# AI4Science-WestlakeU/cindm

Measured on AMD Instinct MI355X. Metric: design samples/sec (1000-step DDPM, composed U-Nets); rel-err vs CPU ref, higher is better.
Workload: dtype f32; 1 GPU; nbody-2 TemporalUnet1D dim=64 horizon=24 attention, single model, batch 256/GPU, 1000 DDPM steps per design (BASELINE configs[1]); unet_evals_per_design=1000, reverse_steps_per_design=1000, parallelism=dp1 (design-sharded, one all-gather of final designs)

## Files before the change

cindm_amd/csrc/cindm_hip.hip:

```cpp
#include "kernels.h"
#include "kernels_dconv.h"
#include "kernels2d.h"
#include "kernels2d_v2.h"
#include "../../include/cindm_hip.h"

#include <hip/hip_ext.h>
#include <cmath>
#include <cstdio>
#include <cstdlib>
#include <cstring>
#include <map>
#include <mutex>
#include <string>
#include <unordered_map>
#include <vector>

using namespace cindm;

static thread_local std::string g_err;
static int fail(const std::string& m) { g_err = m; return -1; }
#define HIPCHK(x) do { hipError_t e_ = (x); if (e_ != hipSuccess) return fail(std::string(#x) + ": " + hipGetErrorString(e_)); } while (0)
#define REQUIRE(c, msg) do { if (!(c)) return fail(msg); } while (0)

extern "C" int cindm_abi_version(void) { return CINDM_ABI_VERSION; }
// ... 120 lines not shown
    }
    const int mid = h->dims[nres];
    rtb("mid_block1", mid, mid);
    if (d.attention) attn("mid_attn", mid);
    rtb("mid_block2", mid, mid);
    cblock("final_conv.0", dim, dim);
    conv("final_conv.1", dim, d.transition_dim, 1);
    return 0;
}

static const OptDef kUnet1dOpts[] = {
    {"mfma_f32", 0, nullptr, OPT_PACK},
    {"local_gn", 1, "CINDM_LOCAL_GN", OPT_PACK},
    {"attn_site", 1, "CINDM_ATTN_SITE", OPT_PACK},
    {"level0", 1, "CINDM_LEVEL0", OPT_PACK},
    {"level1", 1, "CINDM_LEVEL1", OPT_PACK},
    {"ups_last", 1, "CINDM_UPS_LAST", OPT_PACK},
    {"ups_tail", 1, "CINDM_UPS_TAIL", OPT_PACK},
    {"attn_head", 1, "CINDM_ATTN_HEAD", OPT_PACK},
    {"dconv", 1, "CINDM_DCONV", OPT_PACK},
    {"ws_alias", 1, "CINDM_WS_ALIAS", OPT_PACK},
    {"pingpong", 1, "CINDM_PINGPONG", OPT_PACK},
    {"dresample", 2, "CINDM_DRESAMPLE", OPT_PACK},
    {"dconv2", 1, "CINDM_DCONV2", OPT_PACK},
    {"l2_prefetch", 1, "CINDM_L2_PREFETCH", OPT_PACK},
    {"fuse_gather", 1, nullptr, OPT_PACK},
    {"fuse_update", 1, "CINDM_FUSE_UPDATE", OPT_PACK},
    {"taps", 0, "CINDM_TAPS", OPT_PACK},
    {"recover", 1, nullptr, OPT_RUNTIME},
    {"no_exchange", 0, "CINDM_NO_EXCHANGE", OPT_RUNTIME},
    {"tune", 0, "CINDM_TUNE", OPT_RUNTIME},
    {"stress", 0, "CINDM_STRESS", OPT_PACK},
    {"auto_range", 1, "CINDM_AUTO_RANGE", OPT_PACK},
    {"range_fallback", 0, nullptr, OPT_READONLY},
    {"dbg", 0, "CINDM_DBG", OPT_PACK},
};

static void unet1d_plan(cindm_unet1d* h);
extern "C" int cindm_unet1d_set_option(cindm_unet1d* h, const char* key, int32_t value) {
    const int rc = core_set_option(h, key, value);
    if (rc == 1) {
        h->generation = ++g_generation;
        if (std::string(key) == "tune" && h->finalized) unet1d_plan(h);
    }
    return rc < 0 ? -1 : 0;
}
// ... 578 lines not shown
            else DC(3, 4, 0, false);
        }
#undef DC
    }
    E.prof_end();
    hipError_t e = hipGetLastError();
    if (e != hipSuccess && E.err == hipSuccess) E.err = e;
}

static bool dconv_applicable(cindm_unet1d* h, const std::string& p, const Ten& x0, const Ten* x1, int cout) {
    if (!h->O("dconv") || !h->use_h3 || !h->O("local_gn")) return false;
    const int L = x0.L, gw = cout / 8;
    if ((L != 3 && L != 6) || cout % 32 || (gw != 16 && gw != 32 && gw != 64)) return false;
    if (gw == 64 && ((cout / 32) % 2 || h->NX())) return false;
    if (x0.C % 128 || (x1 && (x1->C % 128 || x1->L != L))) return false;
    if (x0.ld != x0.C || (x1 && x1->ld != x1->C)) return false;
    auto w0 = h->packed.find(p + ".blocks.0.block.0"), w1 = h->packed.find(p + ".blocks.1.block.0");
    if (w0 == h->packed.end() || w1 == h->packed.end() || !w0->second.h3 || !w1->second.h3) return false;
    const bool identity = !h->packed.count(p + ".residual_conv");
    if (!identity && !h->packed.count(p + ".residual_conv#h3")) return false;
    const int k0 = x0.C / 128, k1 = x1 ? x1->C / 128 : 0;
    if (w0->second.CinP != (k0 + k1) * 128 || w1->second.CinP != cout || cout % 128) return false;
    return dconv_instantiated(L, k0, k1, !identity) && dconv_instantiated(L, cout / 128, 0, false);
}

static bool dconv2_instantiated(int L, int k0, int k1, bool res, int kb) {
    if (L == 6) return kb == 2 && ((k0 == 1 && k1 == 0 && res) || (k0 == 2 && k1 == 0 && !res) || (k0 == 2 && k1 == 2 && res));
    if (L == 3) return (kb == 4 && ((k0 == 2 && k1 == 0 && res) || (k0 == 4 && k1 == 0 && !res) || (k0 == 4 && k1 == 4 && res))) ||
                       (kb == 2 && k0 == 4 && k1 == 0 && res);
    return false;
}

static Ten emit_rtb_dconv2(Emitter& E, const std::string& p, const Ten& x0, const Ten* x1, int cout) {
    cindm_unet1d* h = E.h;
    const int Bp = (int)E.rows, L = x0.L, S = 48 / L, gw = cout / 8, NT = cout / 32;
    const int tiles = (Bp + S - 1) / S;
    const Packed& w0 = h->packed.at(p + ".blocks.0.block.0");
    const Packed& w1 = h->packed.at(p + ".blocks.1.block.0");
    const bool identity = !h->packed.count(p + ".residual_conv");
    const int k0 = x0.C / 128, k1 = x1 ? x1->C / 128 : 0, kb = cout / 128;
    Ten y0; y0.L = L; y0.C = cout; y0.ld = cout; E.planes(y0);
    Ten out = E.ten(L, cout); E.planes(out);
    unsigned long long* fl = E.xchg((size_t)tiles * NT);
    unsigned long long* xa = gw == 64 ? E.xchg((size_t)tiles * NT * 32) : nullptr;
    unsigned long long* xb = gw == 64 ? E.xchg((size_t)tiles * NT * 32) : nullptr;
    E.need_epoch();
// ... 185 lines not shown
        Emitter::plain(a.src[0], x0);
        if (identity) { a.res = x0.p; a.ldres = x0.ld; } else { a.res = r.p; a.ldres = r.ld; }
    }
    a.e_y = y1.p; a.e_ld = y1.ld; a.e_stats = st1; a.e_P = Pn; a.e_gw = gw; a.e_cnt = cnt;
    a.e_gamma = E.V(p + ".blocks.1.block.2.weight"); a.e_beta = E.V(p + ".blocks.1.block.2.bias");
    a.out = out.p; a.ldo = out.ld;
    if (want_ln) { *ln_out = E.alloc((size_t)Bp * L * (ceil_to(cout, TN) / TN) * 2); a.ln_out = *ln_out; }
    E.launch((identity || fused_res) ? 0 : 1, a);
    E.drop(y0); E.drop(y1); E.drop(k0); E.drop(k1);
    if (fused_res) E.drop(r);
    E.tap(p, out);
    return out;
}

static Ten emit_attn(Emitter& E, const std::string& p, const Ten& x, const float* lnp) {
    cindm_unet1d* h = E.h;
    const int Bp = (int)E.rows, L = x.L, C = x.C;
    const Packed& wq = h->packed.at(p + ".fn.fn.to_qkv");
    const Packed& wo = h->packed.at(p + ".fn.fn.to_out");
    GemmArgs a;
    auto site = h->packed.find(p + ".fn.fn.to_qkv#site");
    if (site != h->packed.end() && site->second.h3 && h->O("attn_head") && !h->NX() && (C == 512 || (C == 256 && (L <= 4 || h->O("attn_head") > 1))) && L <= 16 && x.ld == C) {
        Ten out = E.ten(L, C);
        const int slot = ceil_to(L, 4), S = 16 / slot, groups = (Bp + S - 1) / S;
        unsigned long long* xg = E.xchg((size_t)groups * 2048);
        E.need_epoch();
        ++E.launches;
        Pf pfs;
        E.pf_issue = false;
        E.pf_all(pfs, {&site->second, &h->packed.at(p + ".fn.fn.to_out#site")}, {});
        E.pf_issue = true;
        if (!E.dry) {
            AttnHeadArgs s;
            std::memset(&s, 0, sizeof(s));
            s.pf = pfs;
            s.x = x.p; s.ldx = x.ld; s.out = out.p; s.ldo = out.ld; s.g = E.V(p + ".fn.norm.g");
            s.Wqkv = E.W(site->second); s.Wo = E.W(h->packed.at(p + ".fn.fn.to_out#site")); s.bo = E.B(h->packed.at(p + ".fn.fn.to_out"));
            s.L = L; s.S = S; s.slot = slot; s.Bp = Bp;
            s.xchg = xg; s.epoch = h->ep(); s.err_flag = h->epoch_dev + 1;
            s.stress = h->O("stress");
            s.ph = E.ph_next("attn1d_head<" + std::to_string(C) + "> " + p);
            const dim3 grid(4, (unsigned)groups);
            E.prof_begin(5, 2.0 * Bp * L * 1024.0 * C + (double)Bp * 4 * (2.0 * 32 * 32 * L * 2));
            for (int rep = 0; rep < (E.prof ? Emitter::prof_reps : 1); ++rep) {
                if (C == 256) KLAUNCH(E, attn1d_head_kernel<256>, grid, dim3(256), 0, s);
                else KLAUNCH(E, attn1d_head_kernel<512>, grid, dim3(256), 0, s);
            }
            E.prof_end();
            hipError_t e = hipGetLastError();
            if (e != hipSuccess && E.err == hipSuccess) E.err = e;
        }
        E.tap(p, out);
        return out;
    }
    if (site != h->packed.end() && L <= 32) {
        Ten out = E.ten(L, C);
        ++E.launches;
        Pf pfs;
        E.pf_all(pfs, {&site->second, &h->packed.at(p + ".fn.fn.to_out#site")}, {});
        if (!E.dry) {
            AttnSiteArgs s;
            s.pf = pfs;
            s.x = x.p; s.ldx = x.ld; s.out = out.p; s.ldo = out.ld; s.g = E.V(p + ".fn.norm.g");
            s.Wqkv = E.W(site->second); s.Wo = E.W(h->packed.at(p + ".fn.fn.to_out#site")); s.bo = E.B(h->packed.at(p + ".fn.fn.to_out"));
            s.L = L; s.Bp = Bp;
            s.dbg = 0;
            s.ph = site->second.h3 ? E.ph_next("attn1d_site<" + std::to_string(C) + "> " + p) : PhaseBuf{nullptr, 0};
            const int pack = 1;
            const int NTsel = (L > 16) ? 2 : 1;
            s.slot = (L > 16) ? 32 : ceil_to(L, 4);
            s.S = (L > 16 || !pack) ? 1 : 16 / s.slot;
            const dim3 grid((unsigned)((Bp + s.S - 1) / s.S));
            E.prof_begin(5, 2.0 * Bp * L * 1024.0 * C + (double)Bp * 4 * (2.0 * 32 * 32 * L * 2));
            for (int rep = 0; rep < (E.prof ? Emitter::prof_reps : 1); ++rep) {
#define SITE_LAUNCH(C_, NT_, PF_) KLAUNCH(E, (attn1d_site_kernel<C_, NT_, PF_>), grid, dim3(256), 0, s)
#define SITE_LAUNCH_H3(C_, NT_, PF_) KLAUNCH(E, (attn1d_site_h3_kernel<C_, NT_, PF_>), grid, dim3(256), 0, s)
                if (site->second.h3) {
                    if (NTsel == 2) {
                        if (C == 64) SITE_LAUNCH_H3(64, 2, 2); else if (C == 128) SITE_LAUNCH_H3(128, 2, 3);
                        else if (C == 256) SITE_LAUNCH_H3(256, 2, 3); else SITE_LAUNCH_H3(512, 2, 3);
                    } else {
                        if (C == 64) SITE_LAUNCH_H3(64, 1, 2); else if (C == 128) SITE_LAUNCH_H3(128, 1, 3);
                        else if (C == 256) SITE_LAUNCH_H3(256, 1, 3); else SITE_LAUNCH_H3(512, 1, 3);
                    }
                } else if (NTsel == 2) {
                    if (C == 64) SITE_LAUNCH(64, 2, 4); else if (C == 128) SITE_LAUNCH(128, 2, 4);
                    else if (C == 256) SITE_LAUNCH(256, 2, 4); else SITE_LAUNCH(512, 2, 4);
                } else {
                    if (C == 64) SITE_LAUNCH(64, 1, 4); else if (C == 128) SITE_LAUNCH(128, 1, 4);
// ... 67 lines not shown
    E.tap(p, out);
    return out;
}

static Ten emit_resample(Emitter& E, const std::string& p, const Ten& x, bool up) {
    cindm_unet1d* h = E.h;
    const Packed& w = h->packed.at(p + ".conv");
    const int Lout = up ? x.L * 2 : x.L / 2;
    Ten out = E.ten(Lout, x.C);
    if (h->O("dresample") && h->O("dconv") && w.h3 && x.C == 256 && x.ld == x.C && x.L == (up ? 3 : 6) && w.CinP == x.C && w.T == (up ? 4 : 3)) {
        const int Bp = (int)E.rows, NT = x.C / 32, tiles = (Bp + 15) / 16;
        E.planes(out);
        ++E.launches;
        const bool half = h->O("dresample") >= 2 && NT % 8 == 0 && NT * tiles < 256 && !h->NX();
        int XS = 2;
        while (XS >= 1 && XS < 8 && tiles % (8 / XS) != 0) XS *= 2;
        if (!(XS == 2 || XS == 4) || (half ? 2 * NT : NT) % XS != 0 || (h->O("tune") & 1)) XS = 0;
        Pf pf;
        E.pf_tiled(pf, w, NT);
        if (!E.dry) {
            DresArgs d;
            std::memset(&d, 0, sizeof(d));
            d.pf = pf;
            d.x = x.p; d.ld = x.ld; d.W = reinterpret_cast<const uint4*>(E.W(w)); d.bias = E.B(w); d.nch = w.CinP / 128;
            d.Bp = Bp; d.N = x.C; d.NT = NT; d.out_f32 = out.p; d.ldo = out.ld; d.out_planes = out.pl; d.out_pstride = out.pst;
            d.ph = E.ph_next(std::string("dresample<") + (up ? "up" : "down") + "> " + p);
            d.xs = XS;
            const dim3 grid((unsigned)(half ? 2 * NT : NT), (unsigned)tiles);
            E.prof_begin(up ? 3 : 2, 2.0 * Bp * Lout * x.C * (double)x.C * (up ? 2.0 : 3.0));
            if (E.prof) { E.prof->back().gx = grid.x; E.prof->back().gy = grid.y; E.prof->back().nstage = d.nch; }
            if (half) {
                if (up) KLAUNCH(E, (dresample_kernel<true, 2, 2>), grid, dim3(256), 0, d);
                else KLAUNCH(E, (dresample_kernel<false, 2, 2>), grid, dim3(256), 0, d);
            } else {
                if (up) KLAUNCH(E, (dresample_kernel<true, 2, 1>), grid, dim3(256), 0, d);
                else KLAUNCH(E, (dresample_kernel<false, 2, 1>), grid, dim3(256), 0, d);
            }
            E.prof_end();
            hipError_t e = hipGetLastError();
            if (e != hipSuccess && E.err == hipSuccess) E.err = e;
        }
        E.tap(p, out);
        return out;
    }
    GemmArgs a;
    E.base(a, w, (int)E.rows, x.L, Lout);
    a.pad = 1;
// ... 60 lines not shown
                l.t_ptr = E.t_ptr; l.t_imm = E.t_imm; l.L = L;
                l.ph = E.ph_next("level0_down downs.0");
                E.prof_begin(5, 0.0);
                for (int rep = 0; rep < (E.prof ? Emitter::prof_reps : 1); ++rep) {
                    if (L > 16 && E.rows > 320) KLAUNCH(E, (level0_down_kernel<2, 2>), dim3((unsigned)E.rows), dim3(256), 0, l);
                    else if (L > 16) KLAUNCH(E, level0_down_kernel<2>, dim3((unsigned)E.rows), dim3(256), 0, l);
                    else KLAUNCH(E, level0_down_kernel<1>, dim3((unsigned)E.rows), dim3(256), 0, l);
                }
                E.prof_end();
            }
            if (taps) { E.tap("downs.0.0", h1); E.tap("downs.0.1", h2); }
            E.tap("downs.0.2", sk); E.tap("downs.0.3", dn);
            skips.push_back(sk);
            move_to(dn);
            continue;
        }
        const int lvl1 = h->O("level1");
        if (ind == 1 && lvl1 && h->level1_ok && att && cur.L <= 16 && (cur.L & 1) == 0 && cur.C == 64 && cur.ld == 64 &&
            h->packed.count("downs.1.2.fn.fn.to_qkv#site") && h->packed.at("downs.1.2.fn.fn.to_qkv#site").h3) {
            const int L = cur.L;
            Ten h1, h2;
            if (taps) { h1 = E.ten(L, 128); h2 = E.ten(L, 128); }
            Ten sk = E.ten(L, 128), dn = E.ten(L / 2, 128);
            ++E.launches;
            Pf pfl;
            E.pf_all(pfl, {&h->packed.at("downs.1.0.blocks.0.block.0#lvl"), &h->packed.at("downs.1.0.blocks.1.block.0#lvl"),
                           &h->packed.at("downs.1.1.blocks.0.block.0#lvl"), &h->packed.at("downs.1.1.blocks.1.block.0#lvl"),
                           &h->packed.at("downs.1.0.residual_conv#lvl"), &h->packed.at("downs.1.3.conv#lvl")},
                     {&h->packed.at("downs.1.2.fn.fn.to_qkv#site"), &h->packed.at("downs.1.2.fn.fn.to_out#site")});
            if (!E.dry) {
                Level1Args l;
                std::memset(&l, 0, sizeof(l));
                l.pf = pfl;
                l.x = cur.p; l.h1 = taps ? h1.p : nullptr; l.h2 = taps ? h2.p : nullptr; l.skip = sk.p; l.down = dn.p;
                const char* cv[4] = {"downs.1.0.blocks.0", "downs.1.0.blocks.1", "downs.1.1.blocks.0", "downs.1.1.blocks.1"};
                for (int i = 0; i < 4; ++i) {
                    const std::string cp = cv[i];
                    l.Wc[i] = E.W(h->packed.at(cp + ".block.0#lvl")); l.bc[i] = E.B(h->packed.at(cp + ".block.0"));
                    l.gam[i] = E.V(cp + ".block.2.weight"); l.bet[i] = E.V(cp + ".block.2.bias");
                }
                l.Wr = E.W(h->packed.at("downs.1.0.residual_conv#lvl")); l.br = E.B(h->packed.at("downs.1.0.residual_conv"));
                l.tb0 = h->ttable + h->tb_off.at("downs.1.0"); l.tb1 = h->ttable + h->tb_off.at("downs.1.1"); l.tb_ld = h->tb_ld;
                l.ln_g = E.V("downs.1.2.fn.norm.g"); l.Wqkv = E.W(h->packed.at("downs.1.2.fn.fn.to_qkv#site"));
                l.Wo = E.W(h->packed.at("downs.1.2.fn.fn.to_out#site")); l.bo = E.B(h->packed.at("downs.1.2.fn.fn.to_out"));
                l.Wd = E.W(h->packed.at("downs.1.3.conv#lvl")); l.bd = E.B(h->packed.at("downs.1.3.conv"));
                l.t_ptr = E.t_ptr; l.t_imm = E.t_imm; l.L = L; l.Bp = (int)E.rows;
                l.dbg = 0;
                l.ph = E.ph_next("level1_down downs.1");
                const int S = lvl1 == 1 ? 1 : 2;
                const dim3 grid((unsigned)((E.rows + S - 1) / S));
                E.prof_begin(5, 0.0);
                for (int rep = 0; rep < (E.prof ? Emitter::prof_reps : 1); ++rep) {
                    if (S == 1 && E.rows > 320) KLAUNCH(E, (level1_down_kernel<1, 2>), grid, dim3(256), 0, l);
                    else if (S == 1) KLAUNCH(E, level1_down_kernel<1>, grid, dim3(256), 0, l);
                    else KLAUNCH(E, level1_down_kernel<2>, grid, dim3(256), 0, l);
                }
                E.prof_end();
            }
            if (taps) { E.tap("downs.1.0", h1); E.tap("downs.1.1", h2); }
            E.tap("downs.1.2", sk); E.tap("downs.1.3", dn);
            skips.push_back(sk);
            move_to(dn);
            continue;
        }
        move_to(emit_rtb(E, p + ".0", cur, nullptr, co, false, nullptr));
        move_to(emit_rtb(E, p + ".1", cur, nullptr, co, need_ln(p + ".2", cur.L), &lnp));
        if (att) move_to(emit_attn(E, p + ".2", cur, lnp));
        skips.push_back(cur);
        cur_is_skip = true;
        if (h->packed.count(p + ".3.conv")) move_to(emit_resample(E, p + ".3", cur, false));
// ... 1248 lines not shown
```

cindm_amd/csrc/kernels.h:

```cpp
#pragma once
#include <hip/hip_runtime.h>
#include <stdint.h>
#include <type_traits>

namespace cindm {

typedef float f32x4 __attribute__((ext_vector_type(4)));

__device__ __forceinline__ void permlane16_pair(float v, float& a, float& b) {
    a = v; b = v;
    asm volatile("s_nop 1\n\tv_permlane16_swap_b32_e32 %0, %1\n\ts_nop 1" : "+v"(a), "+v"(b));
}
__device__ __forceinline__ void permlane32_pair(float v, float& a, float& b) {
    a = v; b = v;
    asm volatile("s_nop 1\n\tv_permlane32_swap_b32_e32 %0, %1\n\ts_nop 1" : "+v"(a), "+v"(b));
}
__device__ __forceinline__ float xsum16(float v) { float a, b; permlane16_pair(v, a, b); return a + b; }
__device__ __forceinline__ float xsum32(float v) { float a, b; permlane32_pair(v, a, b); return a + b; }
__device__ __forceinline__ float xmax16(float v) { float a, b; permlane16_pair(v, a, b); return fmaxf(a, b); }
__device__ __forceinline__ float xmax32(float v) { float a, b; permlane32_pair(v, a, b); return fmaxf(a, b); }
template <int CTRL>
__device__ __forceinline__ float dpp_get(float v) {
    return __builtin_bit_cast(float, __builtin_amdgcn_update_dpp(0, __builtin_bit_cast(int, v), CTRL, 0xf, 0xf, false));
}
// ... 556 lines not shown
            for (int ch = 0; ch < nch; ch += 2) {
                stage(ch, bcur, bnxt);
                stage(ch + 1, bnxt, bcur);
            }
        }
    } else {
        if (a.e_y) {
            for (int i = tid; i < ns * 8; i += 256) {
                float m, r;
                merge_stats(a.e_stats + ((size_t)(b0 + i / 8) * 8 + (i & 7)) * a.e_P * 2, a.e_P, a.e_cnt, 1e-5f, m, r);
                tabE[2 * i] = m; tabE[2 * i + 1] = r;
            }
        }
        __syncthreads();
    }

    gemm_epilogue<(T > 0)>(a, acc, Red, tabE, DBG == 8);
}

typedef _Float16 half8 __attribute__((ext_vector_type(8)));
typedef _Float16 half4v __attribute__((ext_vector_type(4)));
constexpr float H3_SCALE = 2048.0f, H3_INV = 1.0f / 2048.0f;

template <int T, int ROWS, int MODE, bool RES = false, int ABL = 0>
__global__ __launch_bounds__(256) void conv_gemm_h3_kernel(const GemmArgs a) {
    constexpr int KC = 128;
    constexpr int PITCH = 272;
    constexpr int F4R = KC / 4;
    constexpr int RPP = 256 / F4R;
    constexpr int NP = (ROWS + RPP - 1) / RPP;
    constexpr int LROWS = NP * RPP;
    constexpr int ZR = LROWS;
    constexpr int PLANE = (LROWS + 1) * PITCH;
    __shared__ __attribute__((aligned(16))) unsigned char Ah[2][2][PLANE];
    __shared__ __attribute__((aligned(16))) float Red[4][TM * LDR];
    __shared__ float tabA[TM * 8 * 2];
    __shared__ float tabE[TM * 8 * 2];

    if (a.dbg == 10) return;
    const int tid = threadIdx.x, lane = tid & 63, w = tid >> 6;
    const int nt = blockIdx.x, mt = blockIdx.y;
    const int b0 = mt * a.spt;
    const int ns = min(a.spt, a.Bp - b0);
    const int rows_out = ns * a.Lout;
    const int rows_in = ns * a.Lin;
    const int t_now = step_scalar(a.t_ptr, a.t_imm);
// ... 289 lines not shown
    const int e = d;
    for (int n = half; n < L; n += 2) {
        float o = 0.f;
#pragma unroll 8
        for (int dd = 0; dd < 32; ++dd) o += ctx[dd * 33 + e] * q[n * 32 + dd];
        att[(row0 + n) * 128 + h * 32 + e] = o;
    }
}

struct AttnSiteArgs {
    const float* x; int ldx;
    float* out; int ldo;
    const float* g;
    const float* Wqkv;
    const float* Wo;
    const float* bo;
    int L;
    int S;
    int slot;
    int Bp;
    int dbg;
    Pf pf;
    PhaseBuf ph;
};

template <int NT>
__device__ __forceinline__ void attn_site_core_range(f32x4 (&qa)[2][NT], f32x4 (&ka)[NT][2], f32x4 (&va)[NT][2], f32x4 (&att)[2][NT],
                                                     int s_begin, int s_end, int nend, int slot, int L, int lq, int lr) {
    const float scale = 0.17677669529663687f;
#pragma unroll
    for (int i = 0; i < 2; ++i)
#pragma unroll
        for (int nt = 0; nt < NT; ++nt) qa[i][nt] *= scale;
    int sid_row[NT][4], sid_col[NT];
#pragma unroll
    for (int nt = 0; nt < NT; ++nt) {
#pragma unroll
        for (int i = 0; i < 4; ++i) { const int n = nt * 16 + lq * 4 + i; sid_row[nt][i] = (n < nend && n % slot < L) ? n / slot : -1; }
        const int n = nt * 16 + lr;
        sid_col[nt] = (n < nend && n % slot < L) ? n / slot : -1;
    }
#pragma unroll
    for (int et = 0; et < 2; ++et)
#pragma unroll
        for (int nt = 0; nt < NT; ++nt) att[et][nt] = f32x4{0.f, 0.f, 0.f, 0.f};
#pragma unroll 1
// ... 399 lines not shown
            const size_t rowc = (n < nend && pn < L) ? row0 + sn * L + pn : row0;
            ex0[nt] = *reinterpret_cast<const float4*>(a.x + rowc * a.ldx + c);
        }
    }
    f32x4 att[2][NT];
    attn_site_core<NT>(qa, ka, va, att, a.dbg == 3 ? 0 : s_here, nend, slot, L, lq, lr);
#pragma unroll
    for (int et = 0; et < 2; ++et)
#pragma unroll
        for (int nt = 0; nt < NT; ++nt) {
            const f32x4 v = att[et][nt];
            half4v hi, lo;
#pragma unroll
            for (int i = 0; i < 4; ++i) { hi[i] = (_Float16)v[i]; lo[i] = (_Float16)((v[i] - (float)hi[i]) * H3_SCALE); }
            const int off = (nt * 16 + lr) * APB + 2 * (w * 32 + et * 16 + lq * 4);
            *reinterpret_cast<half4v*>(&Ap[0][off]) = hi;
            *reinterpret_cast<half4v*>(&Ap[1][off]) = lo;
        }
    __syncthreads();
    PH(2);
    l2_prefetch_late(a.pf, pfr);

    float4 eb[2], ex[2][NT];
    eb[0] = eb0;
#pragma unroll
    for (int nt = 0; nt < NT; ++nt) ex[0][nt] = ex0[nt];
    if (a.dbg != 2)
#pragma unroll
    for (int t = 0; t < TPW; ++t) {
        const int ct = w * TPW + t;
        if (t + WOR - 1 < TPW) {
#pragma unroll
            for (int k = 0; k < 4; ++k)
#pragma unroll
                for (int pl = 0; pl < 2; ++pl)
                    wo[(t + WOR - 1) % WOR][k][pl] = Wo4[(((size_t)(ct + WOR - 1) * 4 + k) * 2 + pl) * 64 + lane];
        }
        if (t + 1 < TPW) {
            const int cn = (ct + 1) * 16 + lq * 4;
            eb[(t + 1) & 1] = *reinterpret_cast<const float4*>(a.bo + cn);
#pragma unroll
            for (int nt = 0; nt < NT; ++nt) {
                const int n = nt * 16 + lr, sn = n / slot, pn = n - sn * slot;
                const size_t rowc = (n < nend && pn < L) ? row0 + sn * L + pn : row0;
                ex[(t + 1) & 1][nt] = *reinterpret_cast<const float4*>(a.x + rowc * a.ldx + cn);
            }
// ... 7 lines not shown
            const half8 wh = __builtin_bit_cast(half8, wo[t % WOR][k][0]), wl = __builtin_bit_cast(half8, wo[t % WOR][k][1]);
#pragma unroll
            for (int nt = 0; nt < NT; ++nt) {
                const int off = (nt * 16 + lr) * APB + k * 64 + lq * 16;
                const half8 ah = *reinterpret_cast<const half8*>(&Ap[0][off]);
                const half8 al = *reinterpret_cast<const half8*>(&Ap[1][off]);
                zM[nt] = __builtin_amdgcn_mfma_f32_16x16x32_f16(wh, ah, zM[nt], 0, 0, 0);
                zL[nt] = __builtin_amdgcn_mfma_f32_16x16x32_f16(wh, al, zL[nt], 0, 0, 0);
                zL[nt] = __builtin_amdgcn_mfma_f32_16x16x32_f16(wl, ah, zL[nt], 0, 0, 0);
            }
        }
        const int c = ct * 16 + lq * 4;
        const float4 b = eb[t & 1];
#pragma unroll
        for (int nt = 0; nt < NT; ++nt) {
            const f32x4 z = zM[nt] + zL[nt] * H3_INV;
            const int n = nt * 16 + lr, sn = n / slot, pn = n - sn * slot;
            if (n < nend && pn < L) {
                const size_t row = row0 + sn * L + pn;
                const float4 xv = ex[t & 1][nt];
                float4 o;
                o.x = z[0] + b.x + xv.x; o.y = z[1] + b.y + xv.y; o.z = z[2] + b.z + xv.z; o.w = z[3] + b.w + xv.w;
                st_out4(a.out, row * a.ldo + c, o, a.pf.wt);
            }
        }
    }
    PH(3);
    l2_prefetch_done(a.pf, pfr);
    PH_FLUSH(a.ph);
}

struct Level0Args {
    const float* x; int F;
    float* h1; float* h2; float* skip; float* down;
    const float* Wc[4]; const float* bc[4]; const float* gam[4]; const float* bet[4];
    const float* Wr; const float* br;
    const float* tb0; const float* tb1; int tb_ld;
    const float* ln_g; const float* Wqkv; const float* Wo; const float* bo;
    const float* Wd; const float* bd;
    const int* t_ptr; int t_imm;
    int L;
    Pf pf; PhaseBuf ph;
    int gB, gcs, gLtot;
};

template <int N>
__device__ __forceinline__ void lvl_wload(const float4* __restrict__ Wt, int lane, float4 (&wr)[N][2]) {
// ... 298 lines not shown
        f32x4 d[1];
        lvl_conv<1, 3, 2, PPB>(wd6, P[0][0], P[0][1], 2, 1, ROWS - 1, lane, d);
        const float4 bd = pbd;
        d[0][0] += bd.x; d[0][1] += bd.y; d[0][2] += bd.z; d[0][3] += bd.w;
        lvl_store<1>(d, a.down + (size_t)b * (L / 2) * C, c0, L / 2, lane, a.pf.wt);
    }
    PH(9);
    l2_prefetch_done(a.pf, pfr);
    PH_FLUSH(a.ph);
}

struct Level1Args {
    const float* x;
    float* h1; float* h2; float* skip; float* down;
    const float* Wc[4]; const float* bc[4]; const float* gam[4]; const float* bet[4];
    const float* Wr; const float* br;
    const float* tb0; const float* tb1; int tb_ld;
    const float* ln_g; const float* Wqkv; const float* Wo; const float* bo;
    const float* Wd; const float* bd;
    const int* t_ptr; int t_imm;
    int L, Bp;
    int dbg;
    Pf pf; PhaseBuf ph;
};

constexpr int LVL_RING = 3;
template <int MT, int KSMAX, int RING = LVL_RING>
struct LvlRing { float4 wr[RING][MT][KSMAX][2]; };

template <int MT, int TAPS, int KS, int KSMAX, int RING>
__device__ __forceinline__ void lvlm_load_tap(LvlRing<MT, KSMAX, RING>& rg, const float4* __restrict__ Wt, int tap, int slot, int lane) {
#pragma unroll
    for (int mt = 0; mt < MT; ++mt)
#pragma unroll
        for (int k = 0; k < KS; ++k)
#pragma unroll
            for (int pl = 0; pl < 2; ++pl) rg.wr[slot][mt][k][pl] = Wt[((((size_t)mt * TAPS + tap) * KS + k) * 2 + pl) * 64 + lane];
}
template <int MT, int TAPS, int KS, int KSMAX, int RING>
__device__ __forceinline__ void lvlm_prefetch(LvlRing<MT, KSMAX, RING>& rg, const float4* __restrict__ Wt, int lane) {
#pragma unroll
    for (int tap = 0; tap < RING - 1; ++tap) if (tap < TAPS) lvlm_load_tap<MT, TAPS, KS, KSMAX>(rg, Wt, tap, tap % RING, lane);
}
template <int MT, int NT, int TAPS, int KS, int PITCHB, int KSMAX, int RMODE = 0, int RING = LVL_RING>
__device__ __forceinline__ void lvlm_conv(LvlRing<MT, KSMAX, RING>& rg, const float4* __restrict__ Wt, const unsigned char* Xh, const unsigned char* Xl,
                                          int tile_rows, int stride, int row0, int maxrow, int lane, f32x4 (&out)[MT][NT]) {
// ... 310 lines not shown
        }
    __syncthreads();
    PH(9);
    if (a.dbg == 5) return;
    f32x4 h3[2][NT];
    lvlm_conv<2, NT, 1, 4, APB, 4>(ring, wbase(a.Wo, 1, 4), Aph, Apl, 16, 1, 0, NP - 1, lane, h3);
    lvlm_prefetch<2, 3, 4, 4>(ring, wbase(a.Wd, 3, 4), lane);
    l2_prefetch_late(a.pf, pfr);
    add4(h3, 15);
#pragma unroll
    for (int mt = 0; mt < 2; ++mt)
#pragma unroll
        for (int nt = 0; nt < NT; ++nt) h3[mt][nt] += h2[mt][nt];
    store(h3, a.skip, L);
    to_planes(h3, P[0][0], P[0][1]);
    __syncthreads();
    PH(10);
    if (a.dbg == 6) return;
    {
        f32x4 d[2][NT];
        lvlm_conv<2, NT, 3, 4, PPB, 4>(ring, wbase(a.Wd, 3, 4), P[0][0], P[0][1], RS, 2, 1, ROWS - 1, lane, d);
        add4(d, 16);
        store(d, a.down, L / 2);
    }
    PH(11);
    l2_prefetch_done(a.pf, pfr);
    PH_FLUSH(a.ph);
}

struct ComposeArgs {
    int mode, W, cs, T, nb, cond_steps, objective, clip;
    float uncond_coef;
    int64_t B;
    int Ltot;
    int F;
    const float* x;
    const float* cond;
    float* pair_in;
    float* single_in;
    const float* pair_eps;
    const float* single_eps;
    const float* sqrt_recip; const float* sqrt_recipm1; const float* sqrt_ac; const float* sqrt_1mac;
    const float* coef1; const float* coef2; const float* logvar;
    const int* t_ptr; int t_imm;
    float* mean_out; float* x0_out; float* eps_out;
    float* x_out;
// ... 1053 lines not shown
```

cindm_amd/csrc/kernels_dconv.h:

```cpp
#pragma once
#include "kernels.h"
#include <type_traits>

namespace cindm {

__device__ __forceinline__ int spin_bound(const int* err_flag, bool forced_short, int full_log2 = 20) {
    const int seen = err_flag ? uniform_word(err_flag) : 0;
    return (forced_short || seen) ? (1 << 8) : (1 << full_log2);
}

struct DSrc {
    const float* f32;
    const uint4* planes;
    size_t pstride;
    int C, ld;
};

struct DconvArgs {
    DSrc src[2];
    const uint4* W; const float* bias;
    int nch;
    int Bp, N, NT;
    int gw;
    const float* gamma; const float* beta;
// ... 64 lines not shown
                g.slot[i] = kq * RPAD + H * S + row;
            }
        }
        g.kstride = g.f32 ? 8 : 192;
        g.second = g.f32 ? 1 : s.pstride;
    };
    auto load_raw = [&](const Stg& g, int j, uint4 (&raw)[3][2]) {
        const size_t ko = (size_t)(4 * j + w) * g.kstride;
#pragma unroll
        for (int i = 0; i < 3; ++i) { raw[i][0] = g.base[i][ko]; raw[i][1] = g.base[i][ko + g.second]; }
    };
    auto store_raw = [&](const Stg& g, int j, const uint4 (&raw)[3][2]) {
        const int kb = (4 * j + w) * 4 * RPAD;
        if (!g.f32) {
#pragma unroll
            for (int i = 0; i < 3; ++i) { Img[0][kb + g.slot[i]] = raw[i][0]; Img[1][kb + g.slot[i]] = raw[i][1]; }
        } else {
#pragma unroll
            for (int i = 0; i < 3; ++i) {
                const float4 v0 = __builtin_bit_cast(float4, raw[i][0]), v1 = __builtin_bit_cast(float4, raw[i][1]);
                const float v[8] = {v0.x, v0.y, v0.z, v0.w, v1.x, v1.y, v1.z, v1.w};
                half8 hi, lo;
#pragma unroll
                for (int e = 0; e < 8; ++e) {
                    hi[e] = (_Float16)v[e];
                    lo[e] = (_Float16)((v[e] - (float)hi[e]) * H3_SCALE);
                }
                Img[0][kb + g.slot[i]] = __builtin_bit_cast(uint4, hi);
                Img[1][kb + g.slot[i]] = __builtin_bit_cast(uint4, lo);
            }
        }
    };

    Stg g0, g1;
    stg_init(a.src[0], g0);
    uint4 raw0[KPW0][3][2];
#pragma unroll
    for (int j = 0; j < KPW0; ++j) load_raw(g0, j, raw0[j]);

    half8 breg[T][2][2];
    const uint4* wbase = a.W + (size_t)nt * a.nch * (T * 4) * 256 + tid;
    auto load_b_tap = [&](int ch, int tap) {
        const uint4* wp = wbase + ((size_t)ch * (T * 4) + tap * 4) * 256;
#pragma unroll
        for (int q = 0; q < 4; ++q) breg[tap][q >> 1][q & 1] = __builtin_bit_cast(half8, wp[q * 256]);
    };
#pragma unroll
    for (int tap = 0; tap < T; ++tap) load_b_tap(0, tap);
    half8 rreg[2][2];
    const uint4* rbase = a.W2 + (size_t)nt * a.nch * 4 * 256 + tid;
// ... 332 lines not shown
                g.slot[i] = kq * RPAD + H * S + row;
            }
        }
        g.kstride = g.f32 ? 8 : 192;
        g.second = g.f32 ? 1 : s.pstride;
    };
    auto load_raw = [&](const Stg& g, int j, uint4 (&raw)[3][2]) {
        const size_t ko = (size_t)(4 * j + w) * g.kstride;
#pragma unroll
        for (int i = 0; i < 3; ++i) { raw[i][0] = g.base[i][ko]; raw[i][1] = g.base[i][ko + g.second]; }
    };
    auto store_raw = [&](bool f32, const int (&slot)[3], int j, const uint4 (&raw)[3][2]) {
        const int kb = (4 * j + w) * 4 * RPAD;
        if (!f32) {
#pragma unroll
            for (int i = 0; i < 3; ++i) { Img[0][kb + slot[i]] = raw[i][0]; Img[1][kb + slot[i]] = raw[i][1]; }
        } else {
#pragma unroll
            for (int i = 0; i < 3; ++i) {
                const float4 v0 = __builtin_bit_cast(float4, raw[i][0]), v1 = __builtin_bit_cast(float4, raw[i][1]);
                const float v[8] = {v0.x, v0.y, v0.z, v0.w, v1.x, v1.y, v1.z, v1.w};
                half8 hi, lo;
#pragma unroll
                for (int e = 0; e < 8; ++e) {
                    hi[e] = (_Float16)v[e];
                    lo[e] = (_Float16)((v[e] - (float)hi[e]) * H3_SCALE);
                }
                Img[0][kb + slot[i]] = __builtin_bit_cast(uint4, hi);
                Img[1][kb + slot[i]] = __builtin_bit_cast(uint4, lo);
            }
        }
    };

    Stg g0, g1;
    stg_init(a.src[0], g0);
    uint4 raw0[KPW0][3][2];
#pragma unroll
    for (int j = 0; j < KPW0; ++j) load_raw(g0, j, raw0[j]);

    constexpr int BD = 1;
    half8 wr[BD][T][2][2];
    const uint4* wbase = a.Wa + (size_t)nt * a.ncha * (T * 4) * 256 + tid;
    const uint4* wbase_b = a.Wb + (size_t)nt * KPWB * (T * 4) * 256 + tid;
    auto load_b_tap = [&](const uint4* wb, int ch, int tap, auto slot_c) {
        constexpr int SL = decltype(slot_c)::value;
#if defined(CINDM_ABL) && (CINDM_ABL & 2)
        ch = 0;
#endif
        const uint4* wp = wb + ((size_t)ch * (T * 4) + tap * 4) * 256;
#pragma unroll
// ... 368 lines not shown
        for (int q = 0; q < 6; ++q)
            if (a.out_f32 && sok[q]) st_out(a.out_f32, (size_t)grow[q] * a.ldo + gn, y[q], 0);
    }
    if (a.out_planes) {
        __syncthreads();
        planes_to_tile(y);
        __syncthreads();
        const uint32_t* tw = reinterpret_cast<const uint32_t*>(Tile);
        for (int i = tid; i < 384; i += 256) {
            const int pl = i >= 192 ? 1 : 0, within = i - pl * 192;
            const int kq = within / 48, row = within - kq * 48;
            const uint4 t4 = *reinterpret_cast<const uint4*>(tw + pl * 48 * TP + row * TP + kq * 4);
            st_out4(a.out_planes, pl * a.out_pstride + ((size_t)mt * a.NT + nt) * 192 + within, t4, a.pf.wt);
        }
    }
    PHX(14);
    l2_prefetch_done(a.pf, pfr);
    PH_FLUSH(a.ph);
}


struct DresArgs {
    const float* x; int ld;
    const uint4* W; const float* bias; int nch;
    int Bp, N, NT;
    float* out_f32; int ldo;
    uint4* out_planes; size_t out_pstride;
    Pf pf;
    PhaseBuf ph;
    int xs;
};

template <bool UP, int KPW, int NH>
__global__ __launch_bounds__(256) void dresample_kernel(const DresArgs a) {
    constexpr int T = UP ? 4 : 3, LIN = UP ? 3 : 6, LOUT = UP ? 6 : 3, S = 16;
    constexpr int TNW = TN / NH, NBW = 2 / NH, RQN = 256 / TNW, LDW = TNW + 1;
    constexpr int RIN = LIN * S, ROUT = LOUT * S, NBLK = LOUT, NQ = ROUT / RQN;
    static_assert(NH == 1 || NH == 2, "32 or 16 columns per workgroup");
    constexpr int KST = 4 * KPW, TP = TNW / 2 + 4;
    __shared__ uint4 Img[2][KST * 4 * RIN];
    __shared__ float Red[4][ROUT * LDW];
    __shared__ uint4 Tile[2 * ROUT * 5];
    PH_DECL;
    PH(0);
    const int tid = threadIdx.x, lane = tid & 63, w = tid >> 6;
    int bx = blockIdx.x, mt = blockIdx.y;
    if (a.xs > 0) {
        const int XS = a.xs, bl = blockIdx.x + gridDim.x * blockIdx.y, xcd = bl & 7, sl = bl >> 3, q4 = gridDim.x / XS;
        bx = (sl % q4) * XS + (xcd & (XS - 1)); mt = (xcd / XS) + (8 / XS) * (sl / q4);
    }
    const int nt = NH == 1 ? bx : bx % a.NT, nbh = NH == 1 ? 0 : bx / a.NT;
    const int b0 = mt * S, ns = min(S, a.Bp - b0);
    const int n = tid & (TNW - 1), rq = tid / TNW, gn = nt * TN + nbh * TNW + n;

    constexpr int NIT = RIN * 4 / 64;
    const float* ibase[NIT];
    int islot[NIT];
#pragma unroll
    for (int i = 0; i < NIT; ++i) {
        const int item = lane + 64 * i, row = item >> 2, kq = item & 3, sm = row % S, pos = row / S;
        ibase[i] = a.x + (size_t)((b0 + min(sm, ns - 1)) * LIN + pos) * a.ld + kq * 8;
        islot[i] = kq * RIN + row;
    }
    float4 raw[KPW][NIT][2];
#pragma unroll
    for (int j = 0; j < KPW; ++j)
#pragma unroll
        for (int i = 0; i < NIT; ++i) {
            const float4* p4 = reinterpret_cast<const float4*>(ibase[i] + (4 * j + w) * 32);
            raw[j][i][0] = p4[0]; raw[j][i][1] = p4[1];
        }
    half8 breg[T][NBW][2];
    const uint4* wbase = a.W + (size_t)nt * a.nch * (T * 4) * 256 + tid;
    auto load_b_tap = [&](int ch, int tap) {
        const uint4* wp = wbase + ((size_t)ch * (T * 4) + tap * 4) * 256;
#pragma unroll
        for (int q = 0; q < 2 * NBW; ++q) breg[tap][q >> 1][q & 1] = __builtin_bit_cast(half8, wp[(NH == 1 ? q : 2 * nbh + q) * 256]);
    };
#pragma unroll
    for (int tap = 0; tap < T; ++tap) load_b_tap(0, tap);
    const float bias_ld = (a.bias ? a.bias : reinterpret_cast<const float*>(a.W))[gn];
    const float bias = a.bias ? bias_ld : 0.f;
    PfRegs pfr;
    l2_prefetch_early(a.pf, pfr);
    __builtin_amdgcn_sched_barrier(0);
    PH(1);

    f32x4 accM[NBLK][NBW], accL[NBLK][NBW];
#pragma unroll
    for (int i = 0; i < NBLK; ++i)
#pragma unroll
        for (int j = 0; j < NBW; ++j) { accM[i][j] = (f32x4){0.f, 0.f, 0.f, 0.f}; accL[i][j] = (f32x4){0.f, 0.f, 0.f, 0.f}; }

    auto kstep = [&](int j, int chn, auto pf) {
        constexpr bool PF = decltype(pf)::value;
        const int kb = (4 * j + w) * 4 * RIN;
#pragma unroll
        for (int i = 0; i < NIT; ++i) {
            const float v[8] = {raw[j][i][0].x, raw[j][i][0].y, raw[j][i][0].z, raw[j][i][0].w, raw[j][i][1].x, raw[j][i][1].y, raw[j][i][1].z, raw[j][i][1].w};
            half8 hi, lo;
#pragma unroll
            for (int e = 0; e < 8; ++e) { hi[e] = (_Float16)v[e]; lo[e] = (_Float16)((v[e] - (float)hi[e]) * H3_SCALE); }
            Img[0][kb + islot[i]] = __builtin_bit_cast(uint4, hi);
            Img[1][kb + islot[i]] = __builtin_bit_cast(uint4, lo);
        }
        const int base = kb + (lane >> 4) * RIN + (lane & 15);
        half8 fh[LIN], fl[LIN];
#pragma unroll
        for (int p = 0; p < LIN; ++p) {
            fh[p] = __builtin_bit_cast(half8, Img[0][base + p * S]);
            fl[p] = __builtin_bit_cast(half8, Img[1][base + p * S]);
        }
#pragma unroll
        for (int tap = 0; tap < T; ++tap) {
#pragma unroll
            for (int lo = 0; lo < LOUT; ++lo) {
                const int num = UP ? lo + 1 - tap : 2 * lo - 1 + tap;
                if (UP && (num & 1)) continue;
                const int p = UP ? num / 2 : num;
                if (num < 0 || p >= LIN) continue;
#pragma unroll
                for (int nb = 0; nb < NBW; ++nb) {
                    accM[lo][nb] = __builtin_amdgcn_mfma_f32_16x16x32_f16(fh[p], breg[tap][nb][0], accM[lo][nb], 0, 0, 0);
                    accL[lo][nb] = __builtin_amdgcn_mfma_f32_16x16x32_f16(fh[p], breg[tap][nb][1], accL[lo][nb], 0, 0, 0);
                }
#pragma unroll
                for (int nb = 0; nb < NBW; ++nb)
// ... 65 lines not shown
                const int sm = r & 15, pos = r >> 4, tile = 2 * mt + (sm >> 3);
                if (tile * 8 >= a.Bp) continue;
                dst = ((size_t)tile * a.NT + nt) * 192 + (nbh * KQW + kq) * 48 + pos * 8 + (sm & 7);
            }
            st_out4(a.out_planes, pl * a.out_pstride + dst, t4, a.pf.wt);
        }
    }
    PH(4);
    l2_prefetch_done(a.pf, pfr);
    PH_FLUSH(a.ph);
}


struct AttnHeadArgs {
    const float* x; int ldx;
    float* out; int ldo;
    const float* g;
    const float* Wqkv; const float* Wo; const float* bo;
    int L, S, slot, Bp;
    unsigned long long* xchg; const int* epoch; int* err_flag;
    Pf pf;
    int stress;
    PhaseBuf ph;
};

template <int C>
__global__ __launch_bounds__(256) void attn1d_head_kernel(const AttnHeadArgs a) {
    constexpr int NP = 16, K32 = C / 32, KPW = K32 / 4, CT4 = C / 64;
    constexpr int YPB = 2 * C + 16;
    constexpr int APB = 2 * 128 + 16;
    constexpr int CH = (C + 255) / 256;
    constexpr int RW = NP / 4;
    __shared__ __attribute__((aligned(16))) unsigned char Yp[2][NP * YPB];
    __shared__ __attribute__((aligned(16))) unsigned char Ap[2][NP * APB];
    __shared__ __attribute__((aligned(16))) float Part[4][24][64];
    PH_DECL;
    PH(0);
    const int tid = threadIdx.x, lane = tid & 63, w = tid >> 6;
    const int lr = lane & 15, lq = lane >> 4;
    const int hd = blockIdx.x, grp = blockIdx.y;
    const int L = a.L, slot = a.slot;
    const int s_here = min(a.S, a.Bp - grp * a.S);
    const int nend = s_here * slot;
    const size_t row0 = (size_t)grp * a.S * L;
    const unsigned tag = (unsigned)uniform_word(a.epoch);
    const int spin_cap = spin_bound(a.err_flag, false, 18);
// ... 195 lines not shown
            for (int j = 0; j < 8; ++j) {
                gq[j] = __hip_atomic_load(gx + tid + 256 * j, __ATOMIC_RELAXED, __HIP_MEMORY_SCOPE_AGENT);
                ok = ok && (unsigned)(gq[j] >> 32) == tag;
            }
            if (__all(ok)) break;
            if (++spins > spin_cap) { if (lane == 0) atomicExch(a.err_flag, 1); break; }
            __builtin_amdgcn_s_sleep(2);
        }
        PH(7);
#pragma unroll
        for (int j = 0; j < 8; ++j) {
            const int idx = tid + 256 * j, h2 = idx >> 9, e = (idx >> 4) & 31, n = idx & 15;
            const float val = __builtin_bit_cast(float, (unsigned)gq[j]);
            const _Float16 hi = (_Float16)val;
            const _Float16 lo = (_Float16)((val - (float)hi) * H3_SCALE);
            const int off = n * APB + 2 * (h2 * 32 + e);
            *reinterpret_cast<_Float16*>(&Ap[0][off]) = hi;
            *reinterpret_cast<_Float16*>(&Ap[1][off]) = lo;
        }
    }
    __syncthreads();
    PH(8);

#pragma unroll
    for (int t = 0; t < TPW; ++t) {
        const int ct = hd * CT4 + w * TPW + t;
        f32x4 zM = f32x4{0.f, 0.f, 0.f, 0.f}, zL = f32x4{0.f, 0.f, 0.f, 0.f};
#pragma unroll
        for (int k = 0; k < 4; ++k) {
            const half8 wh = __builtin_bit_cast(half8, wo[t][k][0]), wl = __builtin_bit_cast(half8, wo[t][k][1]);
            const int off = lr * APB + k * 64 + lq * 16;
            const half8 ah = *reinterpret_cast<const half8*>(&Ap[0][off]);
            const half8 al = *reinterpret_cast<const half8*>(&Ap[1][off]);
            zM = __builtin_amdgcn_mfma_f32_16x16x32_f16(wh, ah, zM, 0, 0, 0);
            zL = __builtin_amdgcn_mfma_f32_16x16x32_f16(wh, al, zL, 0, 0, 0);
            zL = __builtin_amdgcn_mfma_f32_16x16x32_f16(wl, ah, zL, 0, 0, 0);
        }
        const int c = ct * 16 + lq * 4;
        const float4 b = eb[t];
        const f32x4 z = zM + zL * H3_INV;
        const int n = lr, sn = n / slot, pn = n - sn * slot;
        if (n < nend && pn < L) {
            const size_t row = row0 + sn * L + pn;
            const float4 xv = ex[t];
            float4 o;
            o.x = z[0] + b.x + xv.x; o.y = z[1] + b.y + xv.y; o.z = z[2] + b.z + xv.z; o.w = z[3] + b.w + xv.w;
            st_out4(a.out, row * a.ldo + c, o, a.pf.wt);
        }
    }
    PH(9);
    l2_prefetch_done(a.pf, pfr);
    PH_FLUSH(a.ph);
}

}
```

Baseline: 823.6 samples/s.

## Emit pre-split fp16 hi/lo planes from attention and level1 producers for consumers

Result: no change. 823.3 samples/s (-0.0%).

```diff
diff --git a/cindm_amd/csrc/cindm_hip.hip b/cindm_amd/csrc/cindm_hip.hip
--- a/cindm_amd/csrc/cindm_hip.hip
+++ b/cindm_amd/csrc/cindm_hip.hip
@@ -166,6 +166,7 @@
     {"ws_alias", 1, "CINDM_WS_ALIAS", OPT_PACK},
     {"pingpong", 1, "CINDM_PINGPONG", OPT_PACK},
     {"dresample", 2, "CINDM_DRESAMPLE", OPT_PACK},
+    {"src_planes", 1, "CINDM_SRC_PLANES", OPT_PACK},
     {"dconv2", 1, "CINDM_DCONV2", OPT_PACK},
     {"l2_prefetch", 1, "CINDM_L2_PREFETCH", OPT_PACK},
     {"fuse_gather", 1, nullptr, OPT_PACK},
@@ -790,6 +791,10 @@
     const int k0 = x0.C / 128, k1 = x1 ? x1->C / 128 : 0;
     if (w0->second.CinP != (k0 + k1) * 128 || w1->second.CinP != cout || cout % 128) return false;
     return dconv_instantiated(L, k0, k1, !identity) && dconv_instantiated(L, cout / 128, 0, false);
+}
+
+static bool src_planes_wanted(const cindm_unet1d* h, int L, int C) {
+    return h->O("src_planes") && h->use_h3 && h->O("dconv") && h->O("local_gn") && !h->NX() && (L == 3 || L == 6) && C % 128 == 0;
 }
 
 static bool dconv2_instantiated(int L, int k0, int k1, bool res, int kb) {
@@ -1021,6 +1026,7 @@
     auto site = h->packed.find(p + ".fn.fn.to_qkv#site");
     if (site != h->packed.end() && site->second.h3 && h->O("attn_head") && !h->NX() && (C == 512 || (C == 256 && (L <= 4 || h->O("attn_head") > 1))) && L <= 16 && x.ld == C) {
         Ten out = E.ten(L, C);
+        if (src_planes_wanted(h, L, C)) E.planes(out);
         const int slot = ceil_to(L, 4), S = 16 / slot, groups = (Bp + S - 1) / S;
         unsigned long long* xg = E.xchg((size_t)groups * 2048);
         E.need_epoch();
@@ -1038,6 +1044,7 @@
             s.L = L; s.S = S; s.slot = slot; s.Bp = Bp;
             s.xchg = xg; s.epoch = h->ep(); s.err_flag = h->epoch_dev + 1;
             s.stress = h->O("stress");
+            s.out_planes = out.pl; s.out_pstride = out.pst;
             s.ph = E.ph_next("attn1d_head<" + std::to_string(C) + "> " + p);
             const dim3 grid(4, (unsigned)groups);
             E.prof_begin(5, 2.0 * Bp * L * 1024.0 * C + (double)Bp * 4 * (2.0 * 32 * 32 * L * 2));
@@ -1054,6 +1061,7 @@
     }
     if (site != h->packed.end() && L <= 32) {
         Ten out = E.ten(L, C);
+        if (site->second.h3 && C == 256 && L <= 16 && src_planes_wanted(h, L, C)) E.planes(out);
         ++E.launches;
         Pf pfs;
         E.pf_all(pfs, {&site->second, &h->packed.at(p + ".fn.fn.to_out#site")}, {});
@@ -1064,6 +1072,7 @@
             s.Wqkv = E.W(site->second); s.Wo = E.W(h->packed.at(p + ".fn.fn.to_out#site")); s.bo = E.B(h->packed.at(p + ".fn.fn.to_out"));
             s.L = L; s.Bp = Bp;
             s.dbg = 0;
+            s.out_planes = out.pl; s.out_pstride = out.pst;
             s.ph = site->second.h3 ? E.ph_next("attn1d_site<" + std::to_string(C) + "> " + p) : PhaseBuf{nullptr, 0};
             const int pack = 1;
             const int NTsel = (L > 16) ? 2 : 1;
@@ -1177,7 +1186,7 @@
             DresArgs d;
             std::memset(&d, 0, sizeof(d));
             d.pf = pf;
-            d.x = x.p; d.ld = x.ld; d.W = reinterpret_cast<const uint4*>(E.W(w)); d.bias = E.B(w); d.nch = w.CinP / 128;
+            d.x = x.p; d.ld = x.ld; d.xp = x.pl; d.xp_pstride = x.pst; d.W = reinterpret_cast<const uint4*>(E.W(w)); d.bias = E.B(w); d.nch = w.CinP / 128;
             d.Bp = Bp; d.N = x.C; d.NT = NT; d.out_f32 = out.p; d.ldo = out.ld; d.out_planes = out.pl; d.out_pstride = out.pst;
             d.ph = E.ph_next(std::string("dresample<") + (up ? "up" : "down") + "> " + p);
             d.xs = XS;
@@ -1284,6 +1293,7 @@
             Ten h1, h2;
             if (taps) { h1 = E.ten(L, 128); h2 = E.ten(L, 128); }
             Ten sk = E.ten(L, 128), dn = E.ten(L / 2, 128);
+            if (src_planes_wanted(h, L / 2, 128)) E.planes(dn);
             ++E.launches;
             Pf pfl;
             E.pf_all(pfl, {&h->packed.at("downs.1.0.blocks.0.block.0#lvl"), &h->packed.at("downs.1.0.blocks.1.block.0#lvl"),
@@ -1308,6 +1318,7 @@
                 l.Wd = E.W(h->packed.at("downs.1.3.conv#lvl")); l.bd = E.B(h->packed.at("downs.1.3.conv"));
                 l.t_ptr = E.t_ptr; l.t_imm = E.t_imm; l.L = L; l.Bp = (int)E.rows;
                 l.dbg = 0;
+                l.down_planes = dn.pl; l.down_pstride = dn.pst;
                 l.ph = E.ph_next("level1_down downs.1");
                 const int S = lvl1 == 1 ? 1 : 2;
                 const dim3 grid((unsigned)((E.rows + S - 1) / S));
diff --git a/cindm_amd/csrc/kernels.h b/cindm_amd/csrc/kernels.h
--- a/cindm_amd/csrc/kernels.h
+++ b/cindm_amd/csrc/kernels.h
@@ -602,6 +602,27 @@
 typedef _Float16 half4v __attribute__((ext_vector_type(4)));
 constexpr float H3_SCALE = 2048.0f, H3_INV = 1.0f / 2048.0f;
 
+__device__ __forceinline__ void split_h3(float v, _Float16& hi, _Float16& lo) {
+    hi = (_Float16)v;
+    lo = (_Float16)((v - (float)hi) * H3_SCALE);
+}
+
+__device__ __forceinline__ void st_planes_quad(uint4* planes, size_t pstride, int C, int L, int sample, int pos, int c, const float4& v,
+                                               bool ok, int lane, int wt) {
+    const float f[4] = {v.x, v.y, v.z, v.w};
+    _Float16 hi[4], lo[4];
+#pragma unroll
+    for (int i = 0; i < 4; ++i) split_h3(f[i], hi[i], lo[i]);
+    auto pack = [](_Float16 x, _Float16 y) { return (uint32_t)__builtin_bit_cast(uint16_t, x) | ((uint32_t)__builtin_bit_cast(uint16_t, y) << 16); };
+    const uint32_t h0 = pack(hi[0], hi[1]), h1 = pack(hi[2], hi[3]), l0 = pack(lo[0], lo[1]), l1 = pack(lo[2], lo[3]);
+    const bool odd = lane & 16;
+    const uint32_t g0 = (uint32_t)__shfl_xor((int)(odd ? h0 : l0), 16), g1 = (uint32_t)__shfl_xor((int)(odd ? h1 : l1), 16);
+    const uint4 item = odd ? make_uint4(g0, g1, l0, l1) : make_uint4(h0, h1, g0, g1);
+    const int S = 48 / L, c8 = c & ~7, tile = sample / S;
+    const size_t idx = ((size_t)tile * (C >> 5) + (c8 >> 5)) * 192 + ((c8 >> 3) & 3) * 48 + pos * S + (sample - tile * S);
+    if (ok) st_out4(planes, (odd ? pstride : (size_t)0) + idx, item, wt);
+}
+
 template <int T, int ROWS, int MODE, bool RES = false, int ABL = 0>
 __global__ __launch_bounds__(256) void conv_gemm_h3_kernel(const GemmArgs a) {
     constexpr int KC = 128;
@@ -937,6 +958,7 @@
     int dbg;
     Pf pf;
     PhaseBuf ph;
+    uint4* out_planes = nullptr; size_t out_pstride = 0;
 };
 
 template <int NT>
@@ -1382,6 +1404,10 @@
     l2_prefetch_late(a.pf, pfr);
 
     float4 eb[2], ex[2][NT];
+    constexpr bool PLANES = NT == 1 && C == 256;
+    float4 zo[PLANES ? TPW : 1];
+#pragma unroll
+    for (int t = 0; t < (PLANES ? TPW : 1); ++t) zo[t] = make_float4(0.f, 0.f, 0.f, 0.f);
     eb[0] = eb0;
 #pragma unroll
     for (int nt = 0; nt < NT; ++nt) ex[0][nt] = ex0[nt];
@@ -1435,7 +1461,17 @@
                 float4 o;
                 o.x = z[0] + b.x + xv.x; o.y = z[1] + b.y + xv.y; o.z = z[2] + b.z + xv.z; o.w = z[3] + b.w + xv.w;
                 st_out4(a.out, row * a.ldo + c, o, a.pf.wt);
-            }
+                if constexpr (PLANES) zo[t] = o;
+            }
+        }
+    }
+    if constexpr (PLANES) {
+        if (a.out_planes) {
+            const int sn = lr / slot, pn = lr - sn * slot;
+#pragma unroll
+            for (int t = 0; t < TPW; ++t)
+                st_planes_quad(a.out_planes, a.out_pstride, C, L, (int)blockIdx.x * a.S + sn, pn, (w * TPW + t) * 16 + lq * 4, zo[t],
+                               lr < nend && pn < L, lane, a.pf.wt);
         }
     }
     PH(3);
@@ -1780,6 +1816,7 @@
     int L, Bp;
     int dbg;
     Pf pf; PhaseBuf ph;
+    uint4* down_planes; size_t down_pstride;
 };
 
 constexpr int LVL_RING = 3;
@@ -2136,6 +2173,14 @@
         lvlm_conv<2, NT, 3, 4, PPB, 4>(ring, wbase(a.Wd, 3, 4), P[0][0], P[0][1], RS, 2, 1, ROWS - 1, lane, d);
         add4(d, 16);
         store(d, a.down, L / 2);
+        if (a.down_planes) {
+#pragma unroll
+            for (int mt = 0; mt < 2; ++mt)
+#pragma unroll
+                for (int nt = 0; nt < NT; ++nt)
+                    st_planes_quad(a.down_planes, a.down_pstride, C, L / 2, s0 + nt, lr, cl(mt), make_float4(d[mt][nt][0], d[mt][nt][1], d[mt][nt][2], d[mt][nt][3]),
+                                   nt < s_here && lr < L / 2, lane, a.pf.wt);
+        }
     }
     PH(11);
     l2_prefetch_done(a.pf, pfr);
diff --git a/cindm_amd/csrc/kernels_dconv.h b/cindm_amd/csrc/kernels_dconv.h
--- a/cindm_amd/csrc/kernels_dconv.h
+++ b/cindm_amd/csrc/kernels_dconv.h
@@ -110,10 +110,7 @@
                 const float v[8] = {v0.x, v0.y, v0.z, v0.w, v1.x, v1.y, v1.z, v1.w};
                 half8 hi, lo;
 #pragma unroll
-                for (int e = 0; e < 8; ++e) {
-                    hi[e] = (_Float16)v[e];
-                    lo[e] = (_Float16)((v[e] - (float)hi[e]) * H3_SCALE);
-                }
+                for (int e = 0; e < 8; ++e) { _Float16 h, l; split_h3(v[e], h, l); hi[e] = h; lo[e] = l; }
                 Img[0][kb + g.slot[i]] = __builtin_bit_cast(uint4, hi);
                 Img[1][kb + g.slot[i]] = __builtin_bit_cast(uint4, lo);
             }
@@ -492,10 +489,7 @@
                 const float v[8] = {v0.x, v0.y, v0.z, v0.w, v1.x, v1.y, v1.z, v1.w};
                 half8 hi, lo;
 #pragma unroll
-                for (int e = 0; e < 8; ++e) {
-                    hi[e] = (_Float16)v[e];
-                    lo[e] = (_Float16)((v[e] - (float)hi[e]) * H3_SCALE);
-                }
+                for (int e = 0; e < 8; ++e) { _Float16 h, l; split_h3(v[e], h, l); hi[e] = h; lo[e] = l; }
                 Img[0][kb + slot[i]] = __builtin_bit_cast(uint4, hi);
                 Img[1][kb + slot[i]] = __builtin_bit_cast(uint4, lo);
             }
@@ -910,6 +904,7 @@
 
 struct DresArgs {
     const float* x; int ld;
+    const uint4* xp; size_t xp_pstride;
     const uint4* W; const float* bias; int nch;
     int Bp, N, NT;
     float* out_f32; int ldo;
@@ -942,21 +937,32 @@
     const int n = tid & (TNW - 1), rq = tid / TNW, gn = nt * TN + nbh * TNW + n;
 
     constexpr int NIT = RIN * 4 / 64;
-    const float* ibase[NIT];
+    const bool pl_src = a.xp != nullptr;
+    const uint4* ibase[NIT];
     int islot[NIT];
 #pragma unroll
     for (int i = 0; i < NIT; ++i) {
-        const int item = lane + 64 * i, row = item >> 2, kq = item & 3, sm = row % S, pos = row / S;
-        ibase[i] = a.x + (size_t)((b0 + min(sm, ns - 1)) * LIN + pos) * a.ld + kq * 8;
-        islot[i] = kq * RIN + row;
-    }
-    float4 raw[KPW][NIT][2];
+        const int item = lane + 64 * i;
+        if (pl_src) {
+            constexpr int SP = 48 / LIN;
+            const int kq = item / RIN, row = item - kq * RIN, sm = row % S, pos = row / S;
+            const int ntl = (a.Bp + SP - 1) / SP, tile = min(mt * (S / SP) + sm / SP, ntl - 1);
+            ibase[i] = a.xp + (size_t)tile * (a.N >> 5) * 192 + kq * 48 + pos * SP + sm % SP;
+            islot[i] = kq * RIN + row;
+        } else {
+            const int row = item >> 2, kq = item & 3, sm = row % S, pos = row / S;
+            ibase[i] = reinterpret_cast<const uint4*>(a.x + (size_t)((b0 + min(sm, ns - 1)) * LIN + pos) * a.ld + kq * 8);
+            islot[i] = kq * RIN + row;
+        }
+    }
+    const size_t kstride = pl_src ? 192 : 8, second = pl_src ? a.xp_pstride : 1;
+    uint4 raw[KPW][NIT][2];
 #pragma unroll
     for (int j = 0; j < KPW; ++j)
 #pragma unroll
         for (int i = 0; i < NIT; ++i) {
-            const float4* p4 = reinterpret_cast<const float4*>(ibase[i] + (4 * j + w) * 32);
-            raw[j][i][0] = p4[0]; raw[j][i][1] = p4[1];
+            const uint4* p4 = ibase[i] + (size_t)(4 * j + w) * kstride;
+            raw[j][i][0] = p4[0]; raw[j][i][1] = p4[second];
         }
     half8 breg[T][NBW][2];
     const uint4* wbase = a.W + (size_t)nt * a.nch * (T * 4) * 256 + tid;
@@ -983,14 +989,20 @@
     auto kstep = [&](int j, int chn, auto pf) {
         constexpr bool PF = decltype(pf)::value;
         const int kb = (4 * j + w) * 4 * RIN;
-#pragma unroll
-        for (int i = 0; i < NIT; ++i) {
-            const float v[8] = {raw[j][i][0].x, raw[j][i][0].y, raw[j][i][0].z, raw[j][i][0].w, raw[j][i][1].x, raw[j][i][1].y, raw[j][i][1].z, raw[j][i][1].w};
-            half8 hi, lo;
-#pragma unroll
-            for (int e = 0; e < 8; ++e) { hi[e] = (_Float16)v[e]; lo[e] = (_Float16)((v[e] - (float)hi[e]) * H3_SCALE); }
-            Img[0][kb + islot[i]] = __builtin_bit_cast(uint4, hi);
-            Img[1][kb + islot[i]] = __builtin_bit_cast(uint4, lo);
+        if (pl_src) {
+#pragma unroll
+            for (int i = 0; i < NIT; ++i) { Img[0][kb + islot[i]] = raw[j][i][0]; Img[1][kb + islot[i]] = raw[j][i][1]; }
+        } else {
+#pragma unroll
+            for (int i = 0; i < NIT; ++i) {
+                const float4 v0 = __builtin_bit_cast(float4, raw[j][i][0]), v1 = __builtin_bit_cast(float4, raw[j][i][1]);
+                const float v[8] = {v0.x, v0.y, v0.z, v0.w, v1.x, v1.y, v1.z, v1.w};
+                half8 hi, lo;
+#pragma unroll
+                for (int e = 0; e < 8; ++e) { _Float16 h, l; split_h3(v[e], h, l); hi[e] = h; lo[e] = l; }
+                Img[0][kb + islot[i]] = __builtin_bit_cast(uint4, hi);
+                Img[1][kb + islot[i]] = __builtin_bit_cast(uint4, lo);
+            }
         }
         const int base = kb + (lane >> 4) * RIN + (lane & 15);
         half8 fh[LIN], fl[LIN];
@@ -1102,6 +1114,7 @@
     Pf pf;
     int stress;
     PhaseBuf ph;
+    uint4* out_planes; size_t out_pstride;
 };
 
 template <int C>
@@ -1343,6 +1356,9 @@
     __syncthreads();
     PH(8);
 
+    float4 zo[TPW];
+#pragma unroll
+    for (int t = 0; t < TPW; ++t) zo[t] = make_float4(0.f, 0.f, 0.f, 0.f);
 #pragma unroll
     for (int t = 0; t < TPW; ++t) {
         const int ct = hd * CT4 + w * TPW + t;
@@ -1367,7 +1383,15 @@
             float4 o;
             o.x = z[0] + b.x + xv.x; o.y = z[1] + b.y + xv.y; o.z = z[2] + b.z + xv.z; o.w = z[3] + b.w + xv.w;
             st_out4(a.out, row * a.ldo + c, o, a.pf.wt);
-        }
+            zo[t] = o;
+        }
+    }
+    if (a.out_planes) {
+        const int sn = lr / slot, pn = lr - sn * slot;
+#pragma unroll
+        for (int t = 0; t < TPW; ++t)
+            st_planes_quad(a.out_planes, a.out_pstride, C, L, grp * a.S + sn, pn, (hd * CT4 + w * TPW + t) * 16 + lq * 4, zo[t],
+                           lr < nend && pn < L, lane, a.pf.wt);
     }
     PH(9);
     l2_prefetch_done(a.pf, pfr);
```
